# theori-io/nrsc5

Hardware: NVIDIA H100
Metric: cu8 I/Q Msamples/s (higher is better)
Workload: dtype u8/int16/f32

## Files before the change

nrsc5_b200/csrc/engine.cu:

```cuda
#include <cmath>
#include <cstdio>
#include <cstdlib>
#include <cstring>
#include <ctime>
#include <new>
#include <vector>

#include "../../include/nrsc5_b200.h"
#include "chan_feed.h"
#include "common.cuh"
#if defined(NB_EMU)
struct NvtxRange { explicit NvtxRange(const char *) {} };
#else
#include <nvtx3/nvToolsExt.h>
struct NvtxRange {
    explicit NvtxRange(const char *name) { nvtxRangePushA(name); }
    ~NvtxRange() { nvtxRangePop(); }
};
#endif
#include "rs.cuh"
#include "viterbi.cuh"
#include "viterbi_chunk.cuh"
#include "viterbi64.cuh"
#include "front.cuh"
// ... 577 lines not shown
    uint8_t *pinned;
    size_t pinned_cap;
    cudaEvent_t pinned_free;
    long long *avail_rows;
    unsigned avail_rows_pos;
    long long *avail_ring;
    unsigned avail_pos;
    cudaEvent_t reset_done;
    cudaEvent_t fence[64];
    unsigned fence_next;
    StreamState *h_state;
    nrsc5b_stats_t stats;
    unsigned long long last_progress;
    EngineCtl *h_ctl;
    StreamBrief *h_brief;
    uint8_t *xlog;
    size_t xlog_stride;
    ExportHdr *xhdr;
    cudaEvent_t batch_done;
    bool in_flight, batch_decoded;
    bool stalled;
    long long stalled_units;
    struct Staged { int stream; size_t off, n; };
    uint8_t *stage[2];
    size_t stage_cap, stage_fill;
    int stage_cur;
    cudaEvent_t stage_free[2];
    std::vector<Staged> staged;
    std::vector<uint8_t> carry;
    int carry_stream;
    std::vector<long long> staged_units;
    std::vector<uint8_t> unpublished;
    bool direct_push;
    struct Trace {
        unsigned long long batches, passes, decode_passes, flushes, trims, polls_ready, submits_idle;
        double s_flush, s_trim, s_stage_wait, s_submit, s_poll_wait;
    } tr;
    bool trace_on;
    std::vector<void *> allocs;
    int v64_ch;
    nbam::AmState *am_st;
    nbam::AmWork *am_work;
    nbam::AmTables *am_tb;
    uint8_t *am_ring;
    unsigned am_ring_bytes;
    std::vector<long long> am_raw_bytes, am_dec_out;
    nbl2::L2State *l2;
    int profiling;
    cudaEvent_t pev[5];
    double kernel_ms[4];
    unsigned long long kernel_n[4];
};

static const float k_bp_coeff[32] = {
    -0.000685643230099231f, 0.005636964458972216f, 0.009015781804919243f, -0.015486305579543114f,
    -0.035108357667922974f, 0.017446253448724747f, 0.08155813068151474f, 0.007995186373591423f,
    -0.13311293721199036f, -0.0727422907948494f, 0.15914097428321838f, 0.16498781740665436f,
    -0.1324498951435089f, -0.2484012246131897f, 0.051773931831121445f, 0.2821577787399292f,
    0.051773931831121445f, -0.2484012246131897f, -0.1324498951435089f, 0.16498781740665436f,
    0.15914097428321838f, -0.0727422907948494f, -0.13311293721199036f, 0.007995186373591423f,
    0.08155813068151474f, 0.017446253448724747f, -0.035108357667922974f, -0.015486305579543114f,
    0.009015781804919243f, 0.005636964458972216f, -0.000685643230099231f, 0.0f
};

static int upload_tables(int device)
{
    static int done_for = -1;
    if (done_for == device) return 0;
    uint8_t ex[256], lg[256];
    unsigned v = 1;
    lg[0] = 255;
    ex[255] = 0;
    for (int i = 0; i < 255; i++) {
        ex[i] = (uint8_t)v;
        lg[v] = (uint8_t)i;
        v <<= 1;
        if (v & 0x100) v ^= 0x11d;
    }
    CK(cudaMemcpyToSymbol(c_gf_exp, ex, 256));
    CK(cudaMemcpyToSymbol(c_gf_log, lg, 256));
    static const int compat[64] = {
        0, 1, 2, 3, 1, 5, 6, 5, 6, 1, 2, 11, 1, 5, 6, 5, 6, 1, 2, 3, 1, 5, 6, 5, 6, 1, 2, 11, 1, 5, 6, 5,
        6, 1, 2, 3, 1, 5, 6, 5, 6, 1, 2, 11, 1, 5, 6, 5, 6, 1, 2, 3, 1, 5, 6, 5, 6, 1, 2, 11, 1, 5, 6, 5
    };
    CK(cudaMemcpyToSymbol(c_compat_mode, compat, sizeof(compat)));
    short taps[32];
    for (int i = 0; i < 32; i++) taps[i] = (short)(k_bp_coeff[31 - i] * 32767.0f);
    CK(cudaMemcpyToSymbol(c_bp_tap, taps, sizeof(taps)));
    unsigned pn80[3] = { 0, 0, 0 }, reg = 0x3ff;
    for (int i = 0; i < 80; i++) {
        const unsigned b = ((reg >> 9) ^ reg) & 1;
        reg |= b << 11;
        reg >>= 1;
        pn80[i >> 5] |= b << (i & 31);
    }
    CK(cudaMemcpyToSymbol(c_pn80, pn80, sizeof(pn80)));
    done_for = device;
    return 0;
}

template <typename T>
static int dev_alloc(nrsc5b_engine *e, T **ptr, size_t count, bool zero = true)
{
    void *q = nullptr;
    if (cudaMalloc(&q, count * sizeof(T)) != cudaSuccess) return NRSC5B_ENOMEM;
    if (zero && cudaMemset(q, 0, count * sizeof(T)) != cudaSuccess) return NRSC5B_ECUDA;
    e->allocs.push_back(q);
    *ptr = reinterpret_cast<T *>(q);
    return 0;
}

static std::vector<float2> make_twiddles()
{
    std::vector<float2> tw(FFT_TW);
    auto w = [](int m) {
        double a = -2.0 * M_PI * (double)(m % NFFT) / (double)NFFT;
        return make_float2((float)cos(a), (float)sin(a));
    };
    for (int k1 = 0; k1 < 16; k1++)
        for (int t = 0; t < 128; t++) tw[k1 * 128 + t] = w(t * k1);
    for (int k2 = 0; k2 < 16; k2++)
        for (int n3 = 0; n3 < 8; n3++) tw[FFT_TW1 + k2 * 8 + n3] = w(16 * n3 * k2);
    return tw;
}

static void init_state_host(StreamState &st)
{
    memset(&st, 0, sizeof(st));
    st.phase = make_float2(1.0f, 0.0f);
    st.psmi = 1;
    st.state = ST_NONE;
    st.force_state = -1;
}

static void launch_k_stream(nrsc5b_engine *e, int last_pass);

extern "C" int nrsc5b_debug_set(int flags);

extern "C" const char *nrsc5b_version(void) { return "nrsc5_b200 0.1 (sm_90a)"; }

extern "C" int nrsc5b_create(nrsc5b_engine_t **out, const nrsc5b_config_t *cfg)
// ... 1566 lines not shown
```

nrsc5_b200/csrc/front.cuh:

```cuda
#pragma once
#include "pids_crc.cuh"
#include "common.cuh"
#include "fft.cuh"
#include "viterbi_pack.cuh"

namespace nb {

constexpr int FRONT_THREADS = 1024;
constexpr int TEAMS = FRONT_THREADS / 128;
constexpr int MAXREF = 15;
constexpr int IN_BYTES = 4 * NSYM + 28 + 16 + 16;
constexpr int IN_STRIDE = 8704;
constexpr int ACQ_TILE = 4096;

__device__ int g_dbg;

__constant__ int c_compat_mode[64];
__constant__ unsigned c_pn80[3];
__constant__ short c_bp_tap[32];

__device__ __forceinline__ float2 cmulf(float2 a, float2 b)
{
    return make_float2(a.x * b.x - a.y * b.y, a.x * b.y + a.y * b.x);
}
__device__ __forceinline__ float2 cexp_j(float a)
{
    float s, c;
    sincosf(a, &s, &c);
    return make_float2(c, s);
}

__device__ __forceinline__ int partitions_per_band(int psmi)
{
    switch (c_compat_mode[psmi & 63]) {
    case 2: return 11;
    case 3: return 12;
    case 5: case 6: case 11: return 14;
    default: return 10;
    }
}

__device__ void set_state(const DevPtrs &p, const EngineDims &d, int s, int ns)
{
    StreamState &st = p.st[s];
    if (st.state == ns) return;
    if (st.state == ST_FINE) log_reserve(p, d, s, REC_LOST_SYNC, 0);
    if (ns == ST_FINE) {
        float fo = (float)(((double)st.prev_angle - 2 * M_PI * st.cfo) * 744187.5 / (2 * M_PI * NFFT));
        uint8_t *w = log_reserve(p, d, s, REC_SYNC, 8);
        if (w) {
            reinterpret_cast<float *>(w)[0] = fo;
            reinterpret_cast<int *>(w)[1] = st.psmi;
        }
    }
    st.state = ns;
}

constexpr int DEMOD_RUN = 17;
constexpr int TEAM_SMEM = IN_STRIDE + NSYM * (int)sizeof(short2);
struct DemodSmem {
    float2 buf[TEAMS][TEAM_SMEM / sizeof(float2)];
};
static_assert(FFT_SMEM_ELEMS * sizeof(float2) <= TEAM_SMEM && TEAM_SMEM % 16 == 0, "a team's FFT buffer");
static_assert(DEMOD_RUN * FFT_THREADS >= NSYM && DEMOD_RUN % 2 == 1, "a symbol's runs");
struct PrepSmem {
    uint32_t words[ACQ_TILE + 40];
    short2 ytile[ACQ_TILE + 32];
    float2 sums[NSYM];
    float red_mag[FRONT_THREADS];
    int red_idx[FRONT_THREADS];
    float2 red_v[FRONT_THREADS];
};
constexpr int ACQ1_RUN = 3;
constexpr int ACQ1_WORDS = (NSYM + 38 + 3 + 3) / 4 * 4;
static_assert(ACQ1_RUN * FRONT_THREADS >= NSYM + 31 && ACQ1_RUN % 2 == 1, "a tile's runs");
struct Acq1Smem {
    uint32_t words[2][ACQ1_WORDS];
    short2 ytile[NSYM + 32];
    float2 ring[2][NSYM];
    float2 sums[NSYM];
    float2 shape[NCP];
    float red_mag[FRONT_THREADS];
    int red_idx[FRONT_THREADS];
    float2 red_v[FRONT_THREADS];
};
struct PidsSmem {
    int8_t vit[PIDS_LEN * 3];
    uint2 dec[PIDS_LEN + 64];
};
constexpr int ZS = 32;
static_assert(2 * MAXREF <= 32, "a reference slot fits the 5 bits of FrontSmem::ref_plan");
constexpr int EQ_LD = BLK + 1;
constexpr int EQ_MAXPART = 12;
constexpr int EQ_ROWS = 2 * EQ_MAXPART * (PW - 1);
struct SyncSmem {
    float phs[BLK][ZS];
    float2 eph[2 * MAXREF][BLK];
    float smag[2 * MAXREF];
    float cfq[2 * MAXREF];
    union {
        float2 eq[EQ_ROWS][EQ_LD];
        struct {
            int offs[76][22];
            int verdict[76];
            int winner;
        } srch;
    };
    float wred[FRONT_THREADS / 32][2];
    float fb_w[2][MAXREF], fb_xy[2][MAXREF + 1];
    float4 rowc[EQ_ROWS];
    int ref_ok[2 * MAXREF], ref_bc[2 * MAXREF], ref_psmi[2 * MAXREF];
    bool px_on[2];
    long long px_T[2];
    uint8_t *soft_w;
    int do_search;
};
struct BlockSet {
    int samperr;
    int ok;
    float prev_angle, angle;
    float theta;
    float2 phase0, phase;
};
struct FrontSmem {
    float2 tw[FFT_TW];
    float2 nco[NSYM];
    float2 symphase[BLK];
    BlockSet blk;
    float2 zref[BLK][ZS];
    uint8_t ref_plan[128];
    union {
        DemodSmem demod;
        PrepSmem prep;
        Acq1Smem acq1;
        SyncSmem sync;
        PidsSmem pidsq[16];
    } u;
};

__device__ void pids_decode_warp(const DevPtrs &p, const EngineDims &d, int s, int e, PidsSmem &sm, int lane)
{
    const StreamState &st = p.st[s];
    const int bc = st.pids_bc[e];
    const int8_t *pmall = p.pm + (size_t)s * 16 * PM_BLOCK;
    const int8_t PMV[20] = { 10, 2, 18, 6, 14, 8, 16, 0, 12, 4, 11, 3, 19, 7, 15, 9, 17, 1, 13, 5 };
    for (int o = lane; o < PIDS_LEN * 3; o += 32) {
        int8_t v = 0;
        if (o % 6 != 5) {
            unsigned i = (unsigned)bc * 200 + (unsigned)(o - o / 6);
            unsigned part = (unsigned)PMV[i % 20];
            unsigned block = i / 200;
            unsigned k = (i / 20) % 10 + P1_ENC / 320;
            unsigned row = (k * 11) % 32, col = (k * 11 + k / 288) % 36;
            v = pmall[(block * 32 + row) * 720 + part * 36 + col];
        }
        sm.vit[o] = v;
    }
    __syncwarp();
    const int l = lane & 15;
    VitHalf<false> vh;
    vh.init(l);
    vitc_run<false>(vh, sm.vit, PIDS_LEN, PIDS_LEN + 64, 0, PIDS_LEN + 64, 0, sm.dec, lane < 16, l);
    __syncwarp();
    int v = (short)(vh.E & 0xffff), state = 2 * l;
    const int w1 = (short)(vh.O & 0xffff);
    if (w1 > v) { v = w1; state = 2 * l + 1; }
    int v2 = (short)(vh.E >> 16), idx2 = 2 * l + 32;
    const int w3 = (short)(vh.O >> 16);
    if (w3 > v2) { v2 = w3; idx2 = 2 * l + 33; }
    if (v2 > v) { v = v2; state = idx2; }
#pragma unroll
    for (int o = 8; o; o >>= 1) {
        const int ov = __shfl_xor_sync(0xffffffffu, v, o, 16), oi = __shfl_xor_sync(0xffffffffu, state, o, 16);
        if (ov > v || (ov == v && oi < state)) { v = ov; state = oi; }
    }
    if (lane == 0) {
        uint8_t pk[10];
        for (int i = 0; i < 10; i++) pk[i] = 0;
        for (int q = PIDS_LEN + 63; q >= 0; q--) {
            if (q >= 32 && q < 32 + PIDS_LEN) {
                const int i = q - 32;
                const int bit = ((state >> 5) & 1) ^ (int)((c_pn80[i >> 5] >> (i & 31)) & 1u);
                pk[i >> 3] |= (uint8_t)(bit << (7 - (i & 7)));
            }
            state = vitc_prev_head(state, sm.dec, q);
        }
        if (st.pids_rec[e] != 0xffffffffu) {
            uint8_t *w = p.log + (size_t)s * d.log_cap + st.pids_rec[e];
            for (int i = 0; i < 10; i++) w[i] = pk[i];
            w[10] = (uint8_t)pids_crc12_ok(pk);
        }
    }
}

__device__ void front_pids_flush(const DevPtrs &p, const EngineDims &d, int s, PidsSmem *sm, int t)
{
    StreamState &st = p.st[s];
    const int n = st.pids_pending, warp = t >> 5;
    if (warp < n) pids_decode_warp(p, d, s, warp, sm[warp], t & 31);
    __syncthreads();
    if (t == 0) st.pids_pending = 0;
}

constexpr int ACQ_RUN = 5;
static_assert(ACQ_RUN * FRONT_THREADS >= ACQ_TILE + 31, "a tile's runs");
template <int RUN>
__device__ __forceinline__ void acq_tile_input(const EngineDims &d, const uint32_t *words, short2 *ytile, const StreamState &st,
                                               int i0, int L, int t)
{
    const int kb = i0 == 0 ? 31 : 0;
    if (t < kb) ytile[t] = make_short2(st.bp_hist[t][0], st.bp_hist[t][1]);
    const int n = L + 31 - kb;
    if (d.cs16) {
        for (int k = kb + t; k < L + 31; k += FRONT_THREADS) {
            const uint32_t w = words[k + 7];
            ytile[k] = make_short2((short)(w & 0xffff), (short)(w >> 16));
        }
    } else if (RUN * t < n) {
        const int k = kb + min(RUN * t, n - RUN);
        halfband_run<RUN>(words + k, ytile + k);
    }
}

__device__ __forceinline__ float2 acq_bandpass(const short2 *yy)
{
    short accr = 0, acci = 0;
#pragma unroll 5
    for (int k = 1; k < 16; k++) {
        const short2 a = yy[k], b = yy[32 - k];
        accr = (short)(accr + ((((int)a.x + (int)b.x) * c_bp_tap[k]) >> 15));
        acci = (short)(acci + ((((int)a.y + (int)b.y) * c_bp_tap[k]) >> 15));
    }
    const short2 c = yy[16];
    accr = (short)(accr + (((int)c.x * c_bp_tap[16]) >> 15));
    acci = (short)(acci + (((int)c.y * c_bp_tap[16]) >> 15));
    return make_float2(__fdiv_rn((float)accr, 32767.0f), __fdiv_rn((float)acci, -32767.0f));
}

__device__ __forceinline__ void fill_nco(const DevPtrs &p, float2 *nco, float theta, int t, int nthreads = FRONT_THREADS)
{
    for (int j = t; j < NSYM; j += nthreads) {
        float2 e = cexp_j(theta * (float)j);
        if (j < NCP || j >= NFFT) {
            const float w = __ldg(&p.shape[j]);
            e = make_float2(e.x * w, e.y * w);
        }
        nco[j] = e;
    }
}

__device__ __forceinline__ void fill_symphase(float2 *symphase, float theta, float2 phase0, int sym)
{
    double sn, cs;
    sincos((double)theta * (double)(NSYM * sym), &sn, &cs);
    symphase[sym] = cmul(phase0, make_float2((float)cs, (float)sn));
}

__device__ __forceinline__ void block_setup(BlockSet &b, const StreamState &st)
{
    const int adj = NSYM / 2 - b.samperr;
    float angle = b.prev_angle;
    angle = (float)((double)angle - 2 * M_PI * st.cfo);
    const float pre = (float)(-adj) * angle / (float)NFFT;
    const float2 ph = cmulf(st.phase, cexp_j(pre));
    const float theta = angle / (float)NFFT;
    double sn, cs;
    sincos((double)theta * (double)(NSYM * BLK), &sn, &cs);
    const float2 pe = cmulf(ph, make_float2((float)cs, (float)sn));
    const float nrm = sqrtf(pe.x * pe.x + pe.y * pe.y);
    b.angle = angle;
    b.theta = theta;
    b.phase0 = ph;
    b.phase = make_float2(pe.x / nrm, pe.y / nrm);
}

__device__ __forceinline__ void sync_adjust(const DevPtrs &p, int s, int adj, int t)
{
    if (adj == 0) return;
    float *cp = p.cphase + (size_t)s * NFFT;
    for (int i = t; i < SIDE; i += FRONT_THREADS) {
        const int bl = LB0 + i, bu = UB1 - i;
        cp[bl] = (float)((double)cp[bl] - (double)(adj * (bl - NFFT / 2) * 2) * M_PI / NFFT);
        cp[bu] = (float)((double)cp[bu] - (double)(adj * (bu - NFFT / 2) * 2) * M_PI / NFFT);
    }
}

__device__ __forceinline__ void block_commit(const DevPtrs &p, const EngineDims &d, int s, const BlockSet &b, int state_in)
{
    StreamState &st = p.st[s];
// ... 7 lines not shown
        int *wi = reinterpret_cast<int *>(w);
        float *wf = reinterpret_cast<float *>(w);
        wi[0] = state_in; wi[1] = b.samperr; wf[2] = b.angle; wf[3] = b.phase0.x; wf[4] = b.phase0.y; wi[5] = st.cfo;
        wi[6] = (int)(unsigned)(st.start & 0xffffffffLL);
        wi[7] = (int)(st.start >> 32);
    }
}

__device__ int front_prep_begin(const DevPtrs &p, const EngineDims &d, int s, int t)
{
    StreamState &st = p.st[s];
    __shared__ int sh_active;
    if (t == 0) {
        if (st.force_state >= 0) {
            set_state(p, d, s, st.force_state);
            st.force_state = -1;
        }
        const long long avail = *reinterpret_cast<volatile long long *>(&st.in_avail);
        int act = avail >= 2 * (st.start + NACQ);
        if (act && st.state == ST_FINE) {
            const int need = px_need_of(c_compat_mode[st.psmi & 63]);
            if (need & ~d.px_enabled) {
                atomicOr(&p.ctl->px_need, (unsigned)need);
                act = 0;
            }
        }
        st.active = act;
        sh_active = act ? (st.state == ST_FINE ? 1 : 2) : 0;
        if (act) atomicAdd(&p.ctl->progress, 1ull);
    }
    __syncthreads();
    const int mode = sh_active;
    __syncthreads();
    return mode;
}

__device__ void front_acq_tiles(const DevPtrs &p, const EngineDims &d, int s, PrepSmem &sm, int t, int rank, int nranks)
{
    StreamState &st = p.st[s];
    const uint8_t *iq = p.iq + (size_t)s * d.in_stride;
    float2 *tb = p.tbuf + (size_t)s * NACQ;
    const long long start = nranks > 1 ? __ldcg(&st.start) : st.start;
    const uint32_t *iqw = reinterpret_cast<const uint32_t *>(iq);
    for (int i0 = rank * ACQ_TILE; i0 < NACQ; i0 += nranks * ACQ_TILE) {
        const int L = min(ACQ_TILE, NACQ - i0);
        const long long w0 = start + i0 - 38;
        for (int v = t; v < L + 38; v += FRONT_THREADS) {
            const long long a = w0 + v;
            sm.words[v] = a >= 0 ? __ldcg(iqw + a) : (d.cs16 ? 0u : 0x7f7f7f7fu);
        }
        __syncthreads();
        acq_tile_input<ACQ_RUN>(d, sm.words, sm.ytile, st, i0, L, t);
        __syncthreads();
        for (int j = t; j < L; j += FRONT_THREADS) tb[i0 + j] = acq_bandpass(sm.ytile + j);
        if (i0 + L == NACQ && t < 31) {
            const short2 v = sm.ytile[L + t];
            st.bp_hist_next[t][0] = v.x;
            st.bp_hist_next[t][1] = v.y;
        }
        __syncthreads();
    }
}

__device__ void front_acq_corr(const DevPtrs &p, int s, int t, int rank, int nranks)
{
    const float2 *tb = p.tbuf + (size_t)s * NACQ;
    float2 *sums = p.acq_sums + (size_t)s * NSYM;
    const int lo = rank * NSYM / nranks, hi = (rank + 1) * NSYM / nranks;
    for (int i = lo + t; i < hi; i += FRONT_THREADS) {
        float2 acc = make_float2(0.f, 0.f);
        for (int j = 0; j < BLK; j++) {
            const float2 a = __ldcg(&tb[i + j * NSYM]), b = __ldcg(&tb[i + j * NSYM + NFFT]);
            float2 pr = cmulf(a, make_float2(b.x, -b.y));
            acc.x += pr.x;
            acc.y += pr.y;
        }
        sums[i] = acc;
    }
}

__device__ void front_prep_finish(const DevPtrs &p, const EngineDims &d, int s, PrepSmem &sm, float2 *nco, float2 *symphase,
                                  BlockSet &b, int t, int mode)
{
    StreamState &st = p.st[s];
    const int state_in = st.state;
    if (mode == 2) {
        const float2 *gs = p.acq_sums + (size_t)s * NSYM;
        for (int i = t; i < NSYM; i += FRONT_THREADS) sm.sums[i] = __ldcg(&gs[i]);
        if (t < 31) {
            st.bp_hist[t][0] = __ldcg(&st.bp_hist_next[t][0]);
            st.bp_hist[t][1] = __ldcg(&st.bp_hist_next[t][1]);
        }
        __syncthreads();
        float best = -1.0f;
        int besti = 0;
        float2 bestv = make_float2(0.f, 0.f);
        for (int i = t; i < NSYM; i += FRONT_THREADS) {
            float2 v = make_float2(0.f, 0.f);
            for (int j = 0; j < NCP; j++) {
                int q = i + j;
                if (q >= NSYM) q -= NSYM;
                const float2 sv = sm.sums[q];
                const float a = __ldg(&p.shape[j]), b = __ldg(&p.shape[j + NFFT]);
                v.x += (sv.x * a) * b;
                v.y += (sv.y * a) * b;
            }
            const float mag = v.x * v.x + v.y * v.y;
// ... 90 lines not shown
    const int state_in = st.state;
    if (state_in != ST_FINE) {
        const long long start = st.start;
        constexpr int NT = BLK + 1;
        static_assert(NACQ == NT * NSYM, "the window is whole tiles");
        const int woff = (int)((start - 38) & 3);
        static_assert(NSYM % 4 == 0, "tiles start at the same word phase");
        const int nvec = (woff + NSYM + 38 + 3) / 4;
        auto fetch = [&](int T) {
            const long long w0 = start + (long long)T * NSYM - 38;
            const long long w0a = w0 & ~3LL;
            uint4 *dst = reinterpret_cast<uint4 *>(sm.words[T & 1]);
            for (int v = t; v < nvec; v += FRONT_THREADS) {
                const long long a = w0a + 4 * v;
                if (a >= 0) {
#if defined(NB_EMU)
                    dst[v] = *reinterpret_cast<const uint4 *>(iq + 4 * a);
#else
                    asm volatile("cp.async.cg.shared.global [%0], [%1], 16;" ::"r"((unsigned)__cvta_generic_to_shared(dst + v)), "l"(iq + 4 * a) : "memory");
#endif
                } else {
                    const uint32_t z = d.cs16 ? 0u : 0x7f7f7f7fu;
                    dst[v] = make_uint4(z, z, z, z);
                }
            }
#if !defined(NB_EMU)
            asm volatile("cp.async.commit_group;" ::: "memory");
#endif
        };
        for (int i = t; i < NSYM; i += FRONT_THREADS) sm.sums[i] = make_float2(0.f, 0.f);
        if (t < NCP) sm.shape[t] = make_float2(__ldg(&p.shape[t]), __ldg(&p.shape[t + NFFT]));
        fetch(0);
#pragma unroll 1
        for (int T = 0; T <= NT; T++) {
            if (T + 1 < NT) fetch(T + 1);
#if !defined(NB_EMU)
            if (T + 1 < NT) asm volatile("cp.async.wait_group 1;" ::: "memory");
            else asm volatile("cp.async.wait_group 0;" ::: "memory");
#endif
            __syncthreads();
            if (T < NT) acq_tile_input<ACQ1_RUN>(d, sm.words[T & 1] + woff, sm.ytile, st, T * NSYM, NSYM, t);
            if (T >= 2) {
                const float2 *ya = sm.ring[T & 1], *yb = sm.ring[(T - 1) & 1];
                for (int i = t; i < NSYM; i += FRONT_THREADS) {
                    const float2 a = ya[i], b = i + NFFT < NSYM ? ya[i + NFFT] : yb[i + NFFT - NSYM];
                    const float2 pr = cmulf(a, make_float2(b.x, -b.y));
                    sm.sums[i].x += pr.x;
                    sm.sums[i].y += pr.y;
                }
            }
            __syncthreads();
            if (T < NT) {
                float2 *y = sm.ring[T & 1];
                for (int j = t; j < NSYM; j += FRONT_THREADS) y[j] = acq_bandpass(sm.ytile + j);
                if (T == NT - 1 && t < 31) {
                    const short2 v = sm.ytile[NSYM + t];
                    st.bp_hist[t][0] = v.x;
                    st.bp_hist[t][1] = v.y;
                }
            }
        }
        __syncthreads();
        float best = -1.0f;
        int besti = 0;
        float2 bestv = make_float2(0.f, 0.f);
        for (int i = t; i < NSYM; i += FRONT_THREADS) {
            float2 v = make_float2(0.f, 0.f);
            for (int j = 0; j < NCP; j++) {
                int q = i + j;
                if (q >= NSYM) q -= NSYM;
                const float2 sv = sm.sums[q];
                const float2 ab = sm.shape[j];
                v.x += (sv.x * ab.x) * ab.y;
                v.y += (sv.y * ab.x) * ab.y;
            }
            const float mag = v.x * v.x + v.y * v.y;
            if (mag > best) { best = mag; besti = i; bestv = v; }
        }
        sm.red_mag[t] = best; sm.red_idx[t] = besti; sm.red_v[t] = bestv;
        __syncthreads();
        for (int o = FRONT_THREADS / 2; o; o >>= 1) {
            if (t < o) {
                const float m2 = sm.red_mag[t + o];
                const int i2 = sm.red_idx[t + o];
                if (m2 > sm.red_mag[t] || (m2 == sm.red_mag[t] && i2 < sm.red_idx[t])) {
                    sm.red_mag[t] = m2; sm.red_idx[t] = i2; sm.red_v[t] = sm.red_v[t + o];
                }
            }
            __syncthreads();
        }
        if (t == 0) {
            const float2 w = cmulf(sm.red_v[0], cexp_j(-st.prev_angle));
            const float angle_diff = atan2f(w.y, w.x);
            const float factor = (st.prev_angle != 0.0f) ? 0.25f : 1.0f;
            const float angle = st.prev_angle + (angle_diff * factor);
            st.prev_angle = angle;
            b.prev_angle = angle;
            b.samperr = (sm.red_idx[0] + NSYM - 15) % NSYM;
            if (st.state == ST_NONE) st.state = ST_COARSE;
        }
    } else if (t == 0) {
        b.samperr = NSYM / 2 + st.samperr;
        st.samperr = 0;
        const float angle = st.prev_angle + (-st.angle);
        st.angle = 0;
        st.prev_angle = angle;
        b.prev_angle = angle;
// ... 76 lines not shown
    for (int n1 = 1; n1 < 16; n1++) {
        const int j = n1 * 128 + tl;
        v[n1] = cmul(sample_q15(y[j]), nco[j]);
    }
    bar_sync(bar);
    float2 out[2][8];
    fft2048_block<true>(v, out, buf, tw, tl, bar);
    const float2 sp = symphase[sym];

    float2 *dst = p.bins + ((size_t)s * BLK + sym) * NBINS;
    const unsigned plan = ref_plan[tl];
    float2 *zp = zref[sym] + (plan & 31u);
    const unsigned pk = plan >> 5;
    auto put = [&](int c, float2 v, unsigned k) {
        dst[c] = v;
        if (pk == k) *zp = v;
    };
#pragma unroll
    for (int h = 0; h < 2; h++) {
        const int q = tl + 128 * h;
        if (q >= 222) put(q - 222, cmul(out[h][5], sp), 4 * h);
        if (q <= 232) put(q + 34, cmul(out[h][6], sp), 4 * h + 1);
        if (q >= 24) put(q + 243, cmul(out[h][1], sp), 4 * h + 2);
        if (q <= 34) put(q + 499, cmul(out[h][2], sp), 4 * h + 3);
    }
}

__device__ __forceinline__ int ref_bin(int slot)
{
    return slot < MAXREF ? LB0 + PW * slot : UB1 - PW * (slot - MAXREF);
}

__device__ __forceinline__ float atan2_short(float y, float x)
{
    const float ax = fabsf(x), ay = fabsf(y);
    const float mx = fmaxf(ax, ay), mn = fminf(ax, ay);
    const float t = mx > 0.f ? __fdividef(mn, mx) : 0.f;
    const float z = t * t;
    float p = 0.0028340641874819994f;
    p = __fmaf_rn(p, z, -0.016005029901862144f);
    p = __fmaf_rn(p, z, 0.042587608098983765f);
    p = __fmaf_rn(p, z, -0.07495445758104324f);
    p = __fmaf_rn(p, z, 0.10636754333972931f);
    p = __fmaf_rn(p, z, -0.14202570915222168f);
    p = __fmaf_rn(p, z, 0.19992484152317047f);
    p = __fmaf_rn(p, z, -0.3333306610584259f);
    p = __fmaf_rn(p, z, 1.0f);
    float r = p * t;
    if (ay > ax) r = 1.57079637f - r;
    if (x < 0.f) r = 3.14159274f - r;
    return copysignf(r, y);
}

__device__ __forceinline__ void costas_row(float2 *z, float *phs, int zs, float &cfreq, float &cphase, int cfo, float alpha, float beta, bool FAST)
{
    const unsigned pat_pos = (1u << 1) | (1u << 5) | (1u << 6) | (1u << 8) | (1u << 21);
    const unsigned pat_neg = (1u << 0) | (1u << 2) | (1u << 3) | (1u << 4) | (1u << 9) | (1u << 13) | (1u << 14) | (1u << 20) |
                             (1u << 22) | (1u << 31);
    const float cfo_freq = (float)(2 * M_PI * cfo * NCP / NFFT);
    const float PI_F = 3.14159274101257324f;
    const float TWO_PI_HI = 6.28318548202514648f, TWO_PI_LO = -1.74845553e-07f;
    float f = cfreq, ph = cphase;
#pragma unroll 1
    for (int n = 0; n < BLK; n++) {
        const float2 v = z[n * zs];
        float2 rot;
        if (FAST) {
            float sn, cs;
            __sincosf(-ph, &sn, &cs);
            rot = make_float2(cs, sn);
        } else {
            rot = cexp_j(-ph);
        }
        const float2 u = cmulf(v, rot);
        const float error = (FAST ? atan2_short((u.x * u.y) * 2.0f, u.x * u.x - u.y * u.y)
                                  : atan2f((u.x * u.y) * 2.0f, u.x * u.x - u.y * u.y)) * 0.5f;
        phs[n * zs] = ph;
        z[n * zs] = u;
        f += beta * error;
        if (f > 0.5f) f = 0.5f;
        if (f < -0.5f) f = -0.5f;
        ph += (f + cfo_freq) + (alpha * error);
        if (ph >= PI_F) ph = (ph - TWO_PI_HI) - TWO_PI_LO;
        if (ph <= -PI_F) ph = (ph + TWO_PI_HI) + TWO_PI_LO;
    }
    float x = 0;
#pragma unroll 4
    for (int n = 0; n < BLK; n++) x += z[n * zs].x * (float)((int)((pat_pos >> n) & 1u) - (int)((pat_neg >> n) & 1u));
    if (x < 0) {
#pragma unroll 4
        for (int n = 0; n < BLK; n++) {
            phs[n * zs] = (float)((double)phs[n * zs] + M_PI);
            z[n * zs] = make_float2(z[n * zs].x * -1.0f, z[n * zs].y * -1.0f);
        }
        ph = (float)((double)ph + M_PI);
    }
    cfreq = f;
    cphase = ph;
}

__device__ __forceinline__ int needle_bit(int n, unsigned rsid)
{
    const signed char base[BLK] = { 0, 1, 0, 0, 0, 1, 1, -1, 1, 0, 0, 0, -1, 0, 0, -1,
                                    -1, -1, -1, -1, 0, 1, 0, -1, -1, -1, -1, -1, -1, -1, -1, 0 };
    if (n == 10) return (int)(rsid >> 1);
    if (n == 11) return (int)((rsid >> 1) ^ (rsid & 1));
    return base[n];
}

__device__ int ref_find(const float2 *z, int zs, unsigned rsid)
{
    unsigned raw = 0;
    for (int n = 0; n < BLK; n++)
        if (!(z[n * zs].x <= 0)) raw |= 1u << n;
    for (int pass = 0; pass < 2; pass++) {
        for (int n = 0; n < BLK; n++) {
            int i;
            for (i = 0; i < BLK; i++) {
                const int nb_ = needle_bit(i, rsid);
                if (nb_ < 0) continue;
                if (nb_ != (int)((raw >> ((n + i) & 31)) & 1)) break;
            }
            if (i == BLK) return n;
        }
        raw = ~raw;
    }
    return -1;
}

__device__ __forceinline__ float half_pi_wrap(float a, float b)
{
    float dd = a - b;
    while ((double)dd > M_PI / 2) dd = (float)((double)dd - M_PI);
    while ((double)dd < -M_PI / 2) dd = (float)((double)dd + M_PI);
    return dd;
}

__device__ __forceinline__ int8_t soft_demap(float x, float mult)
{
    const float v = fmaxf(fminf(x, 1.0f), -1.0f) * mult;
    int r = __float2int_rz(v);
    const float f = v - (float)r;
    if (f >= 0.5f) r++;
    else if (f <= -0.5f) r--;
    return (int8_t)r;
}

template <bool CL>
__device__ void front_sync(const DevPtrs &p, const EngineDims &d, int s, SyncSmem &sm, float2 (*zref)[ZS], BlockSet &b, int t)
{
    StreamState &st = p.st[s];
    float *cfreq = p.cfreq + (size_t)s * NFFT;
    float *cphase = p.cphase + (size_t)s * NFFT;
    float2 *bins = p.bins + (size_t)s * BLK * NBINS;
    auto ldbin = [](const float2 *q) -> float2 { return CL ? __ldcg(q) : *q; };
    const float loop_bw = 0.05f, damping = 0.70710678f;
    const float denom = 1 + (2 * damping * loop_bw) + (loop_bw * loop_bw);
    const float alpha = (4 * damping * loop_bw) / denom, beta = (4 * loop_bw * loop_bw) / denom;

    int ppb = partitions_per_band(st.psmi);
    int nref = ppb + 1;
    long long sy0 = clock64();
    const bool sy_on = st.state == ST_FINE;
    auto sylap = [&](int k) {
        if (t == 0 && sy_on) {
            const long long c1 = clock64();
            st.sy_cyc[k] += (unsigned long long)(c1 - sy0);
            sy0 = c1;
        }
    };
    auto stage_eq = [&](int first, int stride) {
        const int rows = min(ppb, EQ_MAXPART) * (PW - 1), rows2 = 2 * rows;
        const int dn = stride / rows2, dr = stride - dn * rows2;
        int n = first / rows2, r = first - n * rows2;
#pragma unroll 4
        for (; n < BLK;) {
            const int sb = r >= rows, rr = sb ? r - rows : r;
            const int i = rr / (PW - 1);
            const int ci = sb == 0 ? rr + i + 1 : (NBINS - PW) + rr - (2 * PW - 1) * i;
            sm.eq[r][n] = ldbin(&bins[(size_t)n * NBINS + ci]);
            r += dr;
            n += dn;
            if (r >= rows2) { r -= rows2; n++; }
        }
    };
    const bool pre_staged = st.state == ST_FINE && !(g_dbg & 1);
    if (CL) {
        for (int i = t; i < ZS * BLK; i += FRONT_THREADS) {
            const int slot = i & (ZS - 1), n = i / ZS;
            const int ii = slot < MAXREF ? slot : slot - MAXREF;
            if (slot < 2 * MAXREF && ii < nref) zref[n][slot] = ldbin(&bins[(size_t)n * NBINS + compact_of_bin(ref_bin(slot))]);
        }
        __syncthreads();
    }
    sylap(0);
    if (t < 2 * MAXREF) {
        const int i = t < MAXREF ? t : t - MAXREF;
        if (i < nref) {
            const int b = ref_bin(t);
            float f = cfreq[b], ph = cphase[b];
            costas_row(&zref[0][t], &sm.phs[0][t], ZS, f, ph, 0, alpha, beta, !(g_dbg & 2));
            cfreq[b] = f;
// ... 21 lines not shown
                for (int n = 0; n < BLK; n++) {
                    const int nbit = needle_bit(n, rsid);
                    const int pos = z[n * ZS].x > 0 ? 1 : 0;
                    if (nbit >= 0 && nbit != pos) ok = false;
                    if (!(z[n * ZS].x <= 0)) raw |= 1u << n;
                }
                const unsigned dd = raw ^ (raw << 1);
                auto bit = [&](int n) { return (dd >> n) & 1u; };
                sm.ref_ok[t] = ok;
                sm.ref_bc[t] = (int)(bit(16) << 3 | bit(17) << 2 | bit(18) << 1 | bit(19));
                sm.ref_psmi[t] = (int)(bit(25) << 5 | bit(26) << 4 | bit(27) << 3 | bit(28) << 2 | bit(29) << 1 | bit(30));
            }
        }
        __syncthreads();
        if (t == 0) {
            unsigned good = 0;
            for (int r = 0; r < 2 * MAXREF; r++)
                if (sm.ref_ok[r]) good++;
            sm.do_search = 0;
            if (good >= 4) {
                int mbc = -1, mps = -1;
                for (int v = 0; v < 16; v++) {
                    unsigned nbc = 0, nps = 0;
                    for (int r = 0; r < 2 * MAXREF; r++) {
                        if (!sm.ref_ok[r]) continue;
                        nbc += sm.ref_bc[r] == v;
                        nps += sm.ref_psmi[r] == v;
                    }
                    if (nbc > good / 2) mbc = v;
                    if (nps > good / 2) mps = v;
                }
                if (mbc >= 0 && mps >= 0) {
                    st.bc = mbc;
                    st.psmi = mps;
                    set_state(p, d, s, ST_FINE);
                    l2_enqueue(st, d.l2, 0u, 0, 0);
                    st.started_pm = 0;
                    st.px_total[0] = st.px_total[1] = 0;
                    st.px_started[0] = st.px_started[1] = 0;
                }
            } else if (st.cfo_wait == 0) {
                sm.do_search = 1;
            } else {
                st.cfo_wait--;
            }
        }
        __syncthreads();
        if (sm.do_search) {
            for (int i = t; i < ZS * BLK; i += FRONT_THREADS) {
                const int slot = i & (ZS - 1), n = i / ZS;
                const int ii = slot < MAXREF ? slot : slot - MAXREF;
                if (slot < 2 * MAXREF && ii < nref) bins[(size_t)n * NBINS + compact_of_bin(ref_bin(slot))] = zref[n][slot];
            }
            for (int i = t; i < 76 * 22; i += FRONT_THREADS) sm.srch.offs[i / 22][i % 22] = -1;
            __syncthreads();
            constexpr int SB_BINS = 2 * PW * 2 + 10 * PW;
            constexpr int NSB = 2 * SB_BINS;
            float2 *snap = p.tbuf + (size_t)s * NACQ;
            float *sphs = reinterpret_cast<float *>(p.ydec + (size_t)s * NACQ);
            float fs[4], phsn[4];
            int cfo_of[4], nq = 0, ci = -1, b = 0;
            if (t < NSB) {
                const int upper = t >= SB_BINS;
                b = upper ? (UB1 - 10 * PW - 2 * PW) + (t - SB_BINS) : (LB0 - 2 * PW) + t;
                ci = compact_of_bin(b);
                float f = cfreq[b], ph = cphase[b];
                int ref_i[4];
                for (int step = 0; step <= 10; step++) {
                    const int i = upper ? step : 10 - step;
                    const int cfo = upper ? b - UB1 + PW * i : b - LB0 - PW * i;
                    if (cfo >= -2 * PW && cfo < 2 * PW && nq < 4) {
                        ref_i[nq] = i;
                        cfo_of[nq] = cfo;
                        nq++;
                    }
                }
                for (int q = 0; q < nq; q++) {
                    const int i = ref_i[q], cfo = cfo_of[q];
                    float2 *row = snap + (size_t)q * BLK * NSB + t;
                    const float2 *src = q ? snap + (size_t)(q - 1) * BLK * NSB + t : nullptr;
                    for (int n = 0; n < BLK; n++)
                        row[(size_t)n * NSB] = q ? src[(size_t)n * NSB]
                                                 : (ci >= 0 ? ldbin(&bins[(size_t)n * NBINS + ci]) : make_float2(0.f, 0.f));
                    costas_row(row, sphs + t, NSB, f, ph, cfo, alpha, beta, false);
                    sm.srch.offs[cfo + 2 * PW][2 * i + upper] = ref_find(row, NSB, (unsigned)(30 - i) & 3);
                    for (int n = 0; n < BLK; n++)
                        row[(size_t)n * NSB] = cmulf(row[(size_t)n * NSB], cexp_j(sphs[(size_t)n * NSB + t]));
                    fs[q] = f;
                    phsn[q] = ph;
                }
            }
            __syncthreads();
            if (t < 76) {
                int best = -1;
                unsigned bestn = 0;
                for (int k = 0; k < BLK; k++) {
                    unsigned nv = 0;
                    for (int r = 0; r < 22; r++) nv += sm.srch.offs[t][r] == k;
                    if (nv > bestn) { best = k; bestn = nv; }
                }
                sm.srch.verdict[t] = (best >= 0 && bestn >= 3) ? best : -1;
            }
            __syncthreads();
            if (t == 0) {
                int win = 1 << 20;
                for (int c = 0; c < 76; c++)
                    if (sm.srch.verdict[c] >= 0) { win = c - 2 * PW; break; }
                sm.srch.winner = win;
                if (win < (1 << 20)) {
                    st.keep_extra = ((BLK - sm.srch.verdict[win + 2 * PW]) % BLK) * NSYM;
                    st.cfo += win;
                    st.cfo_wait = 8;
                }
            }
            __syncthreads();
            if (t < NSB) {
                const int win = sm.srch.winner;
                int q = -1;
                for (int k = 0; k < nq; k++)
                    if (cfo_of[k] <= win) q = k;
                if (q >= 0) {
                    cfreq[b] = fs[q];
                    cphase[b] = phsn[q];
                    if (ci >= 0) {
                        const float2 *row = snap + (size_t)q * BLK * NSB + t;
                        for (int n = 0; n < BLK; n++) bins[(size_t)n * NBINS + ci] = row[(size_t)n * NSB];
                    }
                }
            }
        }
        __syncthreads();
    }

    if (st.state == ST_FINE) {
        for (int i = t; i < 2 * MAXREF * BLK; i += FRONT_THREADS) {
            const int slot = i >> 5, n = i & 31;
            const int ii = slot < MAXREF ? slot : slot - MAXREF;
            if (ii < nref) sm.eph[slot][n] = cexp_j(sm.phs[n][slot]);
        }
        const int bc = st.bc;
        int8_t *pm = p.pm + ((size_t)s * 16 + bc) * PM_BLOCK;
        const int rows = min(ppb, EQ_MAXPART) * (PW - 1), rows2 = 2 * rows;
        for (int r = t; r < rows2; r += FRONT_THREADS) {
            const int sb = r >= rows, rr = sb ? r - rows : r;
            const int i = rr / (PW - 1), k = rr - i * (PW - 1) + 1;
            int slot_lo, slot_hi;
            if (sb == 0) { slot_lo = i; slot_hi = i + 1; }
            else { slot_lo = MAXREF + i + 1; slot_hi = MAXREF + i; }
            sm.rowc[r] = make_float4((float)k * sm.smag[slot_hi], (float)(PW - k) * sm.smag[slot_lo],
                                     __int_as_float(slot_hi), __int_as_float(slot_lo));
        }
        sylap(2);
        if (!pre_staged) stage_eq(t, FRONT_THREADS);
        const int cm = c_compat_mode[st.psmi & 63];
        const bool has_px1 = cm == 2 || cm == 3 || cm == 11;
        if (t == 0) {
            sm.px_on[0] = has_px1 && (st.px_started[0] || (bc & 1) == 0);
            sm.px_on[1] = cm == 11 && (st.px_started[1] || (bc & 1) == 0);
            sm.px_T[0] = st.px_total[0];
            sm.px_T[1] = st.px_total[1];
        }
        __syncthreads();
        sylap(3);
        float e_lb = 0.f, e_ub = 0.f;
        if (ppb > EQ_MAXPART) {
            const int xrows = (ppb - EQ_MAXPART) * (PW - 1);
            for (int idx = t; idx < 2 * xrows * BLK; idx += FRONT_THREADS) {
                const int r = idx >> 5, n = idx & (BLK - 1);
                const int sb = r >= xrows, rr = sb ? r - xrows : r;
                const int i = EQ_MAXPART + rr / (PW - 1), k = rr % (PW - 1) + 1;
// ... 275 lines not shown
                c0 = c1;
            }
        };
        int mode = 0;
        if (!CL) {
            if (nb < max_blocks && !st.p1_ready) mode = front_prep_single(p, d, s, sm.u.acq1, sm.nco, sm.symphase, sm.blk, t) ? 1 : 0;
            if (mode == 0) break;
        } else {
            if (owner) {
                if (nb < max_blocks && !st.p1_ready) mode = front_prep_begin(p, d, s, t);
                if (mode == 1) front_prep_finish(p, d, s, sm.u.prep, sm.nco, sm.symphase, sm.blk, t, 1);
            }
            if (owner && t == 0) {
                st.blk_go = mode;
                __threadfence();
            }
            cluster_barrier();
            if (!owner) mode = __ldcg(&st.blk_go);
            if (mode == 0) break;
            if (mode == 2) {
                front_acq_tiles(p, d, s, sm.u.prep, t, rank, C);
                __threadfence();
                cluster_barrier();
                front_acq_corr(p, s, t, rank, C);
                __threadfence();
                cluster_barrier();
                if (owner) {
                    front_prep_finish(p, d, s, sm.u.prep, sm.nco, sm.symphase, sm.blk, t, 2);
                    __threadfence();
                }
                cluster_barrier();
            }
        }
        lap(st.blk_state_in == ST_FINE ? 2 : 1);
        const long long start = CL ? __ldcg(&st.start) : st.start;
        const int samperr = CL ? __ldcg(&st.blk_samperr) : sm.blk.samperr;
        if (CL && !owner) {
            const float theta = __ldcg(&st.theta);
            fill_nco(p, sm.nco, theta, t);
            if (t >= FRONT_THREADS - BLK) fill_symphase(sm.symphase, theta, __ldcg(&st.phase0), t - (FRONT_THREADS - BLK));
            __syncthreads();
        }
#pragma unroll 1
        for (int pass = 0; pass < BLK / (TEAMS * C); pass++)
            front_demod(p, d, s, (pass * C + rank) * TEAMS + team, sm.u.demod, sm.nco, sm.symphase, sm.tw, sm.zref, sm.ref_plan,
                            team, tl, start, samperr);
        if (CL) {
            __threadfence();
            cluster_barrier();
        }
        if (CL && !owner) continue;
        __syncthreads();
        lap(3);
        front_sync<CL>(p, d, s, sm.u.sync, sm.zref, sm.blk, t);
        __syncthreads();
        lap(st.blk_state_in == ST_FINE ? 4 : 5);
    }
    if (CL && !owner) return;
    __syncthreads();
    if (st.pids_pending) {
        const long long c0 = clock64();
        front_pids_flush(p, d, s, sm.u.pidsq, t);
        if (t == 0) {
            st.ph_cyc[0] += (unsigned long long)(clock64() - c0);
            st.ph_n[0]++;
        }
    }
    if (t == 0) {
        StreamBrief b;
        b.start = st.start;
        b.state = st.state;
        b.bc = st.bc;
        b.p1_ready = st.p1_ready;
        b.pad_ = 0;
        p.brief[s] = b;
        const long long avail = *reinterpret_cast<volatile long long *>(&st.in_avail);
        if (last_pass && avail >= 2 * (st.start + NACQ)) atomicAdd(&p.ctl->more, 1u);
    }
}

}
```

Baseline: 180,600.

## Register-blocked band-pass filter, shared-memory search rows, bitmask reference matching

Replaces the per-sample band-pass filter with a register-blocked run filter. Each thread loads a window of samples into registers once and computes several outputs, using compile-time taps instead of constant-memory taps. The CFO search now keeps its working row in shared memory instead of global scratch, and folds the Costas sign flip into the final rotation pass. The reference pattern match becomes a precomputed care/value mask checked with funnel shifts. The goal is less redundant memory traffic and less scalar looping in acquisition and search, at the cost of more registers per thread and a larger shared-memory union member.

After: 184,200, median of 6. Within noise of the previous version (+2.0%).

```diff
diff --git a/nrsc5_b200/csrc/engine.cu b/nrsc5_b200/csrc/engine.cu
--- a/nrsc5_b200/csrc/engine.cu
+++ b/nrsc5_b200/csrc/engine.cu
@@ -653,17 +653,6 @@
     unsigned long long kernel_n[4];
 };
 
-static const float k_bp_coeff[32] = {
-    -0.000685643230099231f, 0.005636964458972216f, 0.009015781804919243f, -0.015486305579543114f,
-    -0.035108357667922974f, 0.017446253448724747f, 0.08155813068151474f, 0.007995186373591423f,
-    -0.13311293721199036f, -0.0727422907948494f, 0.15914097428321838f, 0.16498781740665436f,
-    -0.1324498951435089f, -0.2484012246131897f, 0.051773931831121445f, 0.2821577787399292f,
-    0.051773931831121445f, -0.2484012246131897f, -0.1324498951435089f, 0.16498781740665436f,
-    0.15914097428321838f, -0.0727422907948494f, -0.13311293721199036f, 0.007995186373591423f,
-    0.08155813068151474f, 0.017446253448724747f, -0.035108357667922974f, -0.015486305579543114f,
-    0.009015781804919243f, 0.005636964458972216f, -0.000685643230099231f, 0.0f
-};
-
 static int upload_tables(int device)
 {
     static int done_for = -1;
@@ -685,9 +674,6 @@
         6, 1, 2, 3, 1, 5, 6, 5, 6, 1, 2, 11, 1, 5, 6, 5, 6, 1, 2, 3, 1, 5, 6, 5, 6, 1, 2, 11, 1, 5, 6, 5
     };
     CK(cudaMemcpyToSymbol(c_compat_mode, compat, sizeof(compat)));
-    short taps[32];
-    for (int i = 0; i < 32; i++) taps[i] = (short)(k_bp_coeff[31 - i] * 32767.0f);
-    CK(cudaMemcpyToSymbol(c_bp_tap, taps, sizeof(taps)));
     unsigned pn80[3] = { 0, 0, 0 }, reg = 0x3ff;
     for (int i = 0; i < 80; i++) {
         const unsigned b = ((reg >> 9) ^ reg) & 1;
diff --git a/nrsc5_b200/csrc/front.cuh b/nrsc5_b200/csrc/front.cuh
--- a/nrsc5_b200/csrc/front.cuh
+++ b/nrsc5_b200/csrc/front.cuh
@@ -17,7 +17,6 @@
 
 __constant__ int c_compat_mode[64];
 __constant__ unsigned c_pn80[3];
-__constant__ short c_bp_tap[32];
 
 __device__ __forceinline__ float2 cmulf(float2 a, float2 b)
 {
@@ -74,6 +73,7 @@
 constexpr int ACQ1_RUN = 3;
 constexpr int ACQ1_WORDS = (NSYM + 38 + 3 + 3) / 4 * 4;
 static_assert(ACQ1_RUN * FRONT_THREADS >= NSYM + 31 && ACQ1_RUN % 2 == 1, "a tile's runs");
+static_assert(NSYM % ACQ1_RUN == 0, "a tile's band-pass outputs are whole runs");
 struct Acq1Smem {
     uint32_t words[2][ACQ1_WORDS];
     short2 ytile[NSYM + 32];
@@ -98,14 +98,7 @@
     float2 eph[2 * MAXREF][BLK];
     float smag[2 * MAXREF];
     float cfq[2 * MAXREF];
-    union {
-        float2 eq[EQ_ROWS][EQ_LD];
-        struct {
-            int offs[76][22];
-            int verdict[76];
-            int winner;
-        } srch;
-    };
+    float2 eq[EQ_ROWS][EQ_LD];
     float wred[FRONT_THREADS / 32][2];
     float fb_w[2][MAXREF], fb_xy[2][MAXREF + 1];
     float4 rowc[EQ_ROWS];
@@ -115,6 +108,15 @@
     uint8_t *soft_w;
     int do_search;
 };
+constexpr int SB_BINS = 2 * PW * 2 + 10 * PW;
+constexpr int NSB = 2 * SB_BINS;
+struct SearchSmem {
+    float2 row[BLK][NSB];
+    int8_t offs[76][22];
+    int8_t verdict[76];
+    int winner;
+};
+static_assert(sizeof(SearchSmem) <= sizeof(DemodSmem), "the search fits the phase union as it is");
 struct BlockSet {
     int samperr;
     int ok;
@@ -134,6 +136,7 @@
         PrepSmem prep;
         Acq1Smem acq1;
         SyncSmem sync;
+        SearchSmem srch;
         PidsSmem pidsq[16];
     } u;
 };
@@ -222,19 +225,47 @@
     }
 }
 
-__device__ __forceinline__ float2 acq_bandpass(const short2 *yy)
-{
-    short accr = 0, acci = 0;
-#pragma unroll 5
-    for (int k = 1; k < 16; k++) {
-        const short2 a = yy[k], b = yy[32 - k];
-        accr = (short)(accr + ((((int)a.x + (int)b.x) * c_bp_tap[k]) >> 15));
-        acci = (short)(acci + ((((int)a.y + (int)b.y) * c_bp_tap[k]) >> 15));
-    }
-    const short2 c = yy[16];
-    accr = (short)(accr + (((int)c.x * c_bp_tap[16]) >> 15));
-    acci = (short)(acci + (((int)c.y * c_bp_tap[16]) >> 15));
-    return make_float2(__fdiv_rn((float)accr, 32767.0f), __fdiv_rn((float)acci, -32767.0f));
+constexpr float BP_COEFF[32] = {
+    -0.000685643230099231f, 0.005636964458972216f, 0.009015781804919243f, -0.015486305579543114f,
+    -0.035108357667922974f, 0.017446253448724747f, 0.08155813068151474f, 0.007995186373591423f,
+    -0.13311293721199036f, -0.0727422907948494f, 0.15914097428321838f, 0.16498781740665436f,
+    -0.1324498951435089f, -0.2484012246131897f, 0.051773931831121445f, 0.2821577787399292f,
+    0.051773931831121445f, -0.2484012246131897f, -0.1324498951435089f, 0.16498781740665436f,
+    0.15914097428321838f, -0.0727422907948494f, -0.13311293721199036f, 0.007995186373591423f,
+    0.08155813068151474f, 0.017446253448724747f, -0.035108357667922974f, -0.015486305579543114f,
+    0.009015781804919243f, 0.005636964458972216f, -0.000685643230099231f, 0.0f
+};
+__device__ constexpr int BP_TAP[17] = { 0, -22, 184, 295, -507, -1150, 571, 2672, 261, -4361, -2383, 5214, 5406, -4339, -8139, 1696, 9245 };
+constexpr bool bp_taps_are_the_references()
+{
+    for (int k = 0; k < 17; k++)
+        if (BP_TAP[k] != (short)(BP_COEFF[31 - k] * 32767.0f)) return false;
+    return true;
+}
+static_assert(bp_taps_are_the_references(), "band-pass taps");
+template <int R>
+__device__ __forceinline__ void bandpass_run(const short2 *yy, float2 *out)
+{
+    const short *h = reinterpret_cast<const short *>(yy + 1);
+    int xr[R + 30];
+#pragma unroll
+    for (int q = 0; q < R + 30; q++) xr[q] = h[2 * q];
+    int ar[R];
+#pragma unroll
+    for (int r = 0; r < R; r++) {
+        ar[r] = (xr[r + 15] * BP_TAP[16]) >> 15;
+#pragma unroll
+        for (int k = 1; k < 16; k++) ar[r] += ((xr[r + k - 1] + xr[r + 31 - k]) * BP_TAP[k]) >> 15;
+    }
+#pragma unroll
+    for (int q = 0; q < R + 30; q++) xr[q] = h[2 * q + 1];
+#pragma unroll
+    for (int r = 0; r < R; r++) {
+        int ai = (xr[r + 15] * BP_TAP[16]) >> 15;
+#pragma unroll
+        for (int k = 1; k < 16; k++) ai += ((xr[r + k - 1] + xr[r + 31 - k]) * BP_TAP[k]) >> 15;
+        out[r] = make_float2(__fdiv_rn((float)(short)ar[r], 32767.0f), __fdiv_rn((float)(short)ai, -32767.0f));
+    }
 }
 
 __device__ __forceinline__ void fill_nco(const DevPtrs &p, float2 *nco, float theta, int t, int nthreads = FRONT_THREADS)
@@ -348,7 +379,7 @@
         __syncthreads();
         acq_tile_input<ACQ_RUN>(d, sm.words, sm.ytile, st, i0, L, t);
         __syncthreads();
-        for (int j = t; j < L; j += FRONT_THREADS) tb[i0 + j] = acq_bandpass(sm.ytile + j);
+        for (int j = t; j < L; j += FRONT_THREADS) bandpass_run<1>(sm.ytile + j, tb + i0 + j);
         if (i0 + L == NACQ && t < 31) {
             const short2 v = sm.ytile[L + t];
             st.bp_hist_next[t][0] = v.x;
@@ -545,7 +576,7 @@
             __syncthreads();
             if (T < NT) {
                 float2 *y = sm.ring[T & 1];
-                for (int j = t; j < NSYM; j += FRONT_THREADS) y[j] = acq_bandpass(sm.ytile + j);
+                if (ACQ1_RUN * t < NSYM) bandpass_run<ACQ1_RUN>(sm.ytile + ACQ1_RUN * t, y + ACQ1_RUN * t);
                 if (T == NT - 1 && t < 31) {
                     const short2 v = sm.ytile[NSYM + t];
                     st.bp_hist[t][0] = v.x;
@@ -728,7 +759,7 @@
     return copysignf(r, y);
 }
 
-__device__ __forceinline__ void costas_row(float2 *z, float *phs, int zs, float &cfreq, float &cphase, int cfo, float alpha, float beta, bool FAST)
+__device__ __forceinline__ bool costas_chain(float2 *z, float *phs, int zs, float &cfreq, float &cphase, int cfo, float alpha, float beta, bool FAST)
 {
     const unsigned pat_pos = (1u << 1) | (1u << 5) | (1u << 6) | (1u << 8) | (1u << 21);
     const unsigned pat_neg = (1u << 0) | (1u << 2) | (1u << 3) | (1u << 4) | (1u << 9) | (1u << 13) | (1u << 14) | (1u << 20) |
@@ -763,16 +794,24 @@
     float x = 0;
 #pragma unroll 4
     for (int n = 0; n < BLK; n++) x += z[n * zs].x * (float)((int)((pat_pos >> n) & 1u) - (int)((pat_neg >> n) & 1u));
-    if (x < 0) {
+    cfreq = f;
+    cphase = ph;
+    return x < 0;
+}
+
+__device__ __forceinline__ float turn_pi(float a) { return (float)((double)a + M_PI); }
+__device__ __forceinline__ float2 negate(float2 v) { return make_float2(v.x * -1.0f, v.y * -1.0f); }
+
+__device__ __forceinline__ void costas_row(float2 *z, float *phs, int zs, float &cfreq, float &cphase, int cfo, float alpha, float beta, bool FAST)
+{
+    if (costas_chain(z, phs, zs, cfreq, cphase, cfo, alpha, beta, FAST)) {
 #pragma unroll 4
         for (int n = 0; n < BLK; n++) {
-            phs[n * zs] = (float)((double)phs[n * zs] + M_PI);
-            z[n * zs] = make_float2(z[n * zs].x * -1.0f, z[n * zs].y * -1.0f);
-        }
-        ph = (float)((double)ph + M_PI);
-    }
-    cfreq = f;
-    cphase = ph;
+            phs[n * zs] = turn_pi(phs[n * zs]);
+            z[n * zs] = negate(z[n * zs]);
+        }
+        cphase = turn_pi(cphase);
+    }
 }
 
 __device__ __forceinline__ int needle_bit(int n, unsigned rsid)
@@ -784,21 +823,18 @@
     return base[n];
 }
 
-__device__ int ref_find(const float2 *z, int zs, unsigned rsid)
-{
-    unsigned raw = 0;
-    for (int n = 0; n < BLK; n++)
-        if (!(z[n * zs].x <= 0)) raw |= 1u << n;
+__device__ __forceinline__ int ref_find(unsigned raw, unsigned rsid)
+{
+    unsigned care = 0, val = 0;
+#pragma unroll
+    for (int i = 0; i < BLK; i++) {
+        const int nb_ = needle_bit(i, rsid);
+        if (nb_ >= 0) care |= 1u << i;
+        if (nb_ == 1) val |= 1u << i;
+    }
     for (int pass = 0; pass < 2; pass++) {
-        for (int n = 0; n < BLK; n++) {
-            int i;
-            for (i = 0; i < BLK; i++) {
-                const int nb_ = needle_bit(i, rsid);
-                if (nb_ < 0) continue;
-                if (nb_ != (int)((raw >> ((n + i) & 31)) & 1)) break;
-            }
-            if (i == BLK) return n;
-        }
+        for (int n = 0; n < BLK; n++)
+            if (((__funnelshift_r(raw, raw, n) ^ val) & care) == 0) return n;
         raw = ~raw;
     }
     return -1;
@@ -823,7 +859,8 @@
 }
 
 template <bool CL>
-__device__ void front_sync(const DevPtrs &p, const EngineDims &d, int s, SyncSmem &sm, float2 (*zref)[ZS], BlockSet &b, int t)
+__device__ void front_sync(const DevPtrs &p, const EngineDims &d, int s, SyncSmem &sm, SearchSmem &ss, float2 (*zref)[ZS], BlockSet &b,
+                           int t)
 {
     StreamState &st = p.st[s];
     float *cfreq = p.cfreq + (size_t)s * NFFT;
@@ -951,10 +988,8 @@
                 const int ii = slot < MAXREF ? slot : slot - MAXREF;
                 if (slot < 2 * MAXREF && ii < nref) bins[(size_t)n * NBINS + compact_of_bin(ref_bin(slot))] = zref[n][slot];
             }
-            for (int i = t; i < 76 * 22; i += FRONT_THREADS) sm.srch.offs[i / 22][i % 22] = -1;
+            for (int i = t; i < 76 * 22; i += FRONT_THREADS) ss.offs[i / 22][i % 22] = -1;
             __syncthreads();
-            constexpr int SB_BINS = 2 * PW * 2 + 10 * PW;
-            constexpr int NSB = 2 * SB_BINS;
             float2 *snap = p.tbuf + (size_t)s * NACQ;
             float *sphs = reinterpret_cast<float *>(p.ydec + (size_t)s * NACQ);
             float fs[4], phsn[4];
@@ -974,17 +1009,29 @@
                         nq++;
                     }
                 }
+                float2 *row = &ss.row[0][t];
+#pragma unroll 8
+                for (int n = 0; n < BLK; n++)
+                    row[n * NSB] = ci >= 0 ? ldbin(&bins[(size_t)n * NBINS + ci]) : make_float2(0.f, 0.f);
                 for (int q = 0; q < nq; q++) {
                     const int i = ref_i[q], cfo = cfo_of[q];
-                    float2 *row = snap + (size_t)q * BLK * NSB + t;
-                    const float2 *src = q ? snap + (size_t)(q - 1) * BLK * NSB + t : nullptr;
-                    for (int n = 0; n < BLK; n++)
-                        row[(size_t)n * NSB] = q ? src[(size_t)n * NSB]
-                                                 : (ci >= 0 ? ldbin(&bins[(size_t)n * NBINS + ci]) : make_float2(0.f, 0.f));
-                    costas_row(row, sphs + t, NSB, f, ph, cfo, alpha, beta, false);
-                    sm.srch.offs[cfo + 2 * PW][2 * i + upper] = ref_find(row, NSB, (unsigned)(30 - i) & 3);
-                    for (int n = 0; n < BLK; n++)
-                        row[(size_t)n * NSB] = cmulf(row[(size_t)n * NSB], cexp_j(sphs[(size_t)n * NSB + t]));
+                    const bool inv = costas_chain(row, sphs + t, NSB, f, ph, cfo, alpha, beta, false);
+                    if (inv) ph = turn_pi(ph);
+                    unsigned raw = 0;
+                    for (int n = 0; n < BLK; n++) {
+                        const float x = inv ? row[n * NSB].x * -1.0f : row[n * NSB].x;
+                        if (!(x <= 0)) raw |= 1u << n;
+                    }
+                    ss.offs[cfo + 2 * PW][2 * i + upper] = ref_find(raw, (unsigned)(30 - i) & 3);
+                    float2 *out = snap + (size_t)q * BLK * NSB + t;
+#pragma unroll 8
+                    for (int n = 0; n < BLK; n++) {
+                        const float a = sphs[(size_t)n * NSB + t];
+                        const float2 z = row[n * NSB];
+                        const float2 v = cmulf(inv ? negate(z) : z, cexp_j(inv ? turn_pi(a) : a));
+                        row[n * NSB] = v;
+                        out[(size_t)n * NSB] = v;
+                    }
                     fs[q] = f;
                     phsn[q] = ph;
                 }
@@ -995,26 +1042,26 @@
                 unsigned bestn = 0;
                 for (int k = 0; k < BLK; k++) {
                     unsigned nv = 0;
-                    for (int r = 0; r < 22; r++) nv += sm.srch.offs[t][r] == k;
+                    for (int r = 0; r < 22; r++) nv += ss.offs[t][r] == k;
                     if (nv > bestn) { best = k; bestn = nv; }
                 }
-                sm.srch.verdict[t] = (best >= 0 && bestn >= 3) ? best : -1;
+                ss.verdict[t] = (best >= 0 && bestn >= 3) ? best : -1;
             }
             __syncthreads();
             if (t == 0) {
                 int win = 1 << 20;
                 for (int c = 0; c < 76; c++)
-                    if (sm.srch.verdict[c] >= 0) { win = c - 2 * PW; break; }
-                sm.srch.winner = win;
+                    if (ss.verdict[c] >= 0) { win = c - 2 * PW; break; }
+                ss.winner = win;
                 if (win < (1 << 20)) {
-                    st.keep_extra = ((BLK - sm.srch.verdict[win + 2 * PW]) % BLK) * NSYM;
+                    st.keep_extra = ((BLK - ss.verdict[win + 2 * PW]) % BLK) * NSYM;
                     st.cfo += win;
                     st.cfo_wait = 8;
                 }
             }
             __syncthreads();
             if (t < NSB) {
-                const int win = sm.srch.winner;
+                const int win = ss.winner;
                 int q = -1;
                 for (int k = 0; k < nq; k++)
                     if (cfo_of[k] <= win) q = k;
@@ -1396,7 +1443,7 @@
         if (CL && !owner) continue;
         __syncthreads();
         lap(3);
-        front_sync<CL>(p, d, s, sm.u.sync, sm.zref, sm.blk, t);
+        front_sync<CL>(p, d, s, sm.u.sync, sm.u.srch, sm.zref, sm.blk, t);
         __syncthreads();
         lap(st.blk_state_in == ST_FINE ? 4 : 5);
     }
```
